# Junacik99/opengl-ray-tracer

Hardware: AMD Instinct MI355X
Metric: Mrays/sec + FPS @1920x1080, car scene (4122 shapes), 1/2/4/8 GPUs (higher is better)
Workload: dtype f32

## Files before the change

### opengl-ray-tracer_amd/csrc/rt_device.h

```cpp
#pragma once

#include <hip/hip_runtime.h>
#include <stdint.h>

namespace rtd {

struct GeoRec {
    int type, idx;
    float f[18];
};
static_assert(sizeof(GeoRec) == 80, "GeoRec is 5 float4");

struct PrimRec {
    float f[15];
    int st;
};
static_assert(sizeof(PrimRec) == 64, "PrimRec is 4 float4");
__device__ __forceinline__ int prim_type(const PrimRec& g) { return g.st & 3; }

struct V {
    float x, y, z;
};
__host__ __device__ __forceinline__ V mk(float x, float y, float z) { return V{x, y, z}; }
__host__ __device__ __forceinline__ V operator+(V a, V b) { return V{a.x + b.x, a.y + b.y, a.z + b.z}; }
// ... 29 lines not shown
    int S, N, I;
    int max_stack;
    V cam_pos, cam_front, cam_right, cam_up;
    float plane_w, plane_h;
    V light_pos, light_color;
    float resX, resY;
    int maxBounces, useBVH, useFresnel, useMT;
    int width, height, y0, stripe, period, out_rows;
    char* __restrict__ dst;
    size_t pitch;
    unsigned long long* __restrict__ stats;
    unsigned long long* __restrict__ tile_times;
    int tiles_x, tiles;
    const int* __restrict__ tile_order;
    int lane_k, lane_k_mode;
    int heavy_k, heavy_parts;
    unsigned* __restrict__ tile_cost;
    int cost_time;
    unsigned long long* __restrict__ heavy_acc;
    unsigned* __restrict__ sched_hist;
    int lane_from_depth;
    int shadow_lane_from;
    int root_ok;
    float root_lo[3], root_hi[3];
    int lane_stack;
    float4* __restrict__ tail_queue;
    int* __restrict__ tail_px;
    int* __restrict__ tail_count;
    int* __restrict__ tail_count_next;
    int tail_from;
    int tail_rx, tail_regions;
    int tail_counters;
    int tail_max_lanes;
    int rgb;
    float shadow_off;
    int ss;
};

__device__ __forceinline__ int image_row(const KParams& kp, int r) {
    return kp.y0 + r + (r / kp.stripe) * (kp.period - kp.stripe);
}

__device__ __forceinline__ Ray get_ray(const KParams& kp, float ndcX, float ndcY) {
    V p = ((kp.cam_pos + kp.cam_front) + (ndcX * kp.plane_w / 2.0f) * kp.cam_right) +
          (ndcY * kp.plane_h / 2.0f) * kp.cam_up;
    return Ray{kp.cam_pos, normalize(p - kp.cam_pos)};
}

struct Hit {
    int type;
    V p;
};

__device__ __forceinline__ Hit intersect(const GeoRec& g, const Ray& r, int use_mt) {
    Hit h{NONE, V{0.f, 0.f, 0.f}};
    const float* f = g.f;
    if (g.type == 0) {
        V c = mk(f[0], f[1], f[2]);
        V oc = r.o - c;
        float aa = dot(r.d, r.d);
        float bb = 2.0f * dot(r.d, oc);
        float cc = dot(oc, oc) - f[3] * f[3];
        float D = bb * bb - 4.0f * aa * cc;
        if (D > 0.0f) {
            float sD = __builtin_sqrtf(D);
            float t1 = (-bb - sD) / (2.0f * aa);
// ... 163 lines not shown
```

### opengl-ray-tracer_amd/csrc/rt_kernels.hip

```cpp
#include <hip/hip_runtime.h>

#include <algorithm>
#include <chrono>
#include <climits>
#include <cmath>
#include <cstdio>
#include <cstdlib>
#include <cstring>
#include <functional>
#include <limits>
#include <atomic>
#include <memory>
#include <new>
#include <thread>
#include <vector>

#include "../../include/rt_api.h"
#include "accel.h"
#include "accel_math.h"
#include "lbvh.h"
#include "rt_device.h"
#include "group_wait.h"
#include "rt_internal.h"

using namespace rtd;

namespace {

constexpr int kBlock = 256;
constexpr int kTileW = 32;
constexpr int kTileH = 8;
constexpr int kMaxStack = 64;
constexpr int kRing = 1024;
constexpr int kLeafScan = 8;

enum {
    ST_PIXELS = 0, ST_CLOSEST, ST_SHADOW, ST_NODES,
    ST_BVH0, ST_BVH1, ST_BVH2, ST_BVH3,
    ST_BR0, ST_BR1, ST_BR2, ST_BR3,
    ST_UPD, ST_HITS, ST_COUNT
};


__device__ GeoRec pack_geo(const FlatShape& s, int si) {
    GeoRec g;
    for (int k = 0; k < 18; ++k) g.f[k] = 0.f;
    g.type = s.type;
    g.idx = si;
    if (s.type == RT_SPHERE) {
        g.f[0] = s.sphereCenter.x; g.f[1] = s.sphereCenter.y; g.f[2] = s.sphereCenter.z;
        g.f[3] = s.sphereRadius;
    } else {
        V n = mk(s.planeNormal.x, s.planeNormal.y, s.planeNormal.z);
        g.f[0] = n.x; g.f[1] = n.y; g.f[2] = n.z; g.f[3] = s.planeD;
        if (s.type == RT_WALL) {
            g.f[4] = s.wallStart.x; g.f[5] = s.wallStart.y; g.f[6] = s.wallStart.z;
// ... 831 lines not shown
        const int ci = k.code[i], cj = k.code[j];
        k.t[i] = sw ? tj : ti, k.t[j] = sw ? ti : tj;
        k.code[i] = sw ? cj : ci, k.code[j] = sw ? ci : cj;
    };
    cx(0, 1), cx(2, 3), cx(4, 5), cx(6, 7), cx(0, 2), cx(1, 3), cx(4, 6), cx(5, 7), cx(1, 2), cx(5, 6);
    cx(0, 4), cx(1, 5), cx(2, 6), cx(3, 7), cx(2, 4), cx(3, 5), cx(1, 2), cx(3, 4), cx(5, 6);
    return k;
}
__device__ __forceinline__ int pick_code8(const Kids8& k, int i) {
    int r = k.code[0];
#pragma unroll
    for (int s2 = 1; s2 < 8; ++s2) r = i == s2 ? k.code[s2] : r;
    return r;
}
__device__ __forceinline__ float pick_t8(const Kids8& k, int i) {
    float r = k.t[0];
#pragma unroll
    for (int s2 = 1; s2 < 8; ++s2) r = i == s2 ? k.t[s2] : r;
    return r;
}

__device__ __forceinline__ int pick_code(const Kids4& k, int i) {
    return i == 0 ? k.code[0] : i == 1 ? k.code[1] : i == 2 ? k.code[2] : k.code[3];
}
__device__ __forceinline__ float pick_t(const Kids4& k, int i) {
    return i == 0 ? k.t[0] : i == 1 ? k.t[1] : i == 2 ? k.t[2] : k.t[3];
}

__device__ __forceinline__ unsigned short f_bf16_down(float t) {
    return static_cast<unsigned short>(__float_as_uint(t) >> 16);
}
__device__ __forceinline__ float bf16_f(unsigned short b) { return __uint_as_float(static_cast<unsigned>(b) << 16); }

template <bool SHADOW, bool COUNT = false, bool WSTAT = false, bool MT = false, bool FLAT_SHADOW = false>
__device__ void lane_walk(const AccelPtrs& A, const Ray& r, bool active, float lim_shadow, Best& b, bool& shadow,
                          int* stk, unsigned short* stt, int stride, int cap, WalkCount& wc, int sg = 1,
                          int si = 0) {
    if (A.N <= 0 || !active) return;
    const V inv = inv_dir(r.d);
    const bool fast = A.boxes_finite && aabb_fast_ok(r.o, inv);
    const rta::RayC c = ray_c<MT>(r, A);
    float tl = rta::t_limit(SHADOW ? lim_shadow : b.d, c.rdl);
    int sp = 0, cur = A.troot;
    const int capo = cap * stride;
    bool have = true;
    bool ovf = false;
    int pcap = min(cap, A.scene_stack) * stride;
    unsigned fm = 0;
    if (!use_scene(A, fast, c)) {
        have = enter_root(A, r, inv, c, tl, cur);
        pcap = capo;
    } else if (A.nfew > 0) {
        fm = few_mask(A, r, inv);
    }
    int start = 0, count = 0;
    if (sg > 1) {
        const float tl0 = SHADOW ? tl : INFINITY;
        int ss = sg;
        while (have && ss > 1) {
            const unsigned uc = static_cast<unsigned>(cur);
            if (uc & (kLeaf | kItem)) break;
            if (COUNT) wc.nodes++;
            if (uc & kTopLeaf) {
                if (count > 0) break;
                const int4 lf = A.tleaf[uc & 0x0fffffffu];
                start = lf.x;
                count = lf.y;
                have = lf.z != kNoChild;
                cur = lf.z;
            } else if (uc & kLocal) {
                if constexpr (!MT && kWide8) {
                    const Kids8 w = sort8(wide_kids<MT>(A, uc, c, tl0, true), wide_kids_hi<MT>(A, uc, c, tl0, true));
                    int h = 0;
#pragma unroll
                    for (int s2 = 0; s2 < 8; ++s2) h += w.t[s2] < INFINITY;
                    if (h == 0) {
                        have = false;
                    } else if (h >= ss) {
                        for (int q = si + ss; q < h; q += ss) {
                            if (sp < pcap) {
                                stk[sp] = pick_code8(w, q);
                                stt[sp] = f_bf16_down(pick_t8(w, q));
                                sp += stride;
                            } else {
                                ovf = true;
                            }
                        }
// ... 17 lines not shown
                                stk[sp] = pick_code(w, si + ss);
                                stt[sp] = f_bf16_down(pick_t(w, si + ss));
                                sp += stride;
                            } else {
                                ovf = true;
                            }
                        }
                        cur = pick_code(w, si);
                        ss = 1;
                    } else {
                        const int p = si * h / ss, lo = (p * ss + h - 1) / h, hi = ((p + 1) * ss + h - 1) / h;
                        cur = pick_code(w, p);
                        si -= lo;
                        ss = hi - lo;
                    }
                }
            } else {
                const Kids k = ref_kids(A, uc, r, inv, c, tl0, true, fast);
                if (k.ha && k.hb) {
                    const bool a_first = !(k.tb < k.ta);
                    const int p = si * 2 / ss, lo = (p * ss + 1) / 2, hi = ((p + 1) * ss + 1) / 2;
                    cur = (p == 0) == a_first ? k.ca : k.cb;
                    si -= lo;
                    ss = hi - lo;
                } else if (k.ha || k.hb) {
                    cur = k.ha ? k.ca : k.cb;
                } else {
                    have = false;
                }
            }
        }
    }
    if (!have) cur = kNoChild;
    bool ended = false;
    for (;;) {
        bool stop = ended;
        for (;;) {
            if (__ballot(!stop && count == 0) == 0) break;
            if (!stop && cur == kNoChild) {
                if (sp == 0) {
                    if (ovf) {
                        ovf = false;
                        pcap = capo;
                        if (!enter_root(A, r, inv, c, tl, cur)) cur = kNoChild;
                    }
                    if (cur == kNoChild) {
                        ended = count == 0;
                        stop = true;
                    }
                } else {
                    sp -= stride;
                    const int pc = stk[sp];
                    cur = bf16_f(stt[sp]) > tl ? kNoChild : pc;
                }
            }
            const unsigned uc = static_cast<unsigned>(cur);
            stop = stop || (cur != kNoChild && count > 0 && (uc & (kTopLeaf | kLeaf)));
            if (stop || cur == kNoChild) continue;
            if (COUNT) wc.nodes++;
            if (WSTAT && first_active()) wc.wnodes++;
            cur = kNoChild;
            if (uc & kLocal) {
                if (uc & kLeaf) {
                    start = static_cast<int>((uc >> 6) & 0x3fffffu);
                    count = static_cast<int>(uc & 0x3fu);
                    if (uc & kItem) count = ((fm >> (count >> 3)) & 1u) ? (count & 7) : 0;
                } else {
                    auto push = [&](float t, int code) {
// ... 26 lines not shown
                        const bool vf = vt < w.t[0];
                        push(vf ? w.t[0] : vt, vf ? w.code[0] : vc);
                        w.t[0] = vf ? vt : w.t[0];
                        w.code[0] = vf ? vc : w.code[0];
                    }
                    if (w.t[0] < INFINITY) cur = w.code[0];
                }
            } else if ((uc & (kTopLeaf | kItem)) == (kTopLeaf | kItem)) {
                int s0, n0;
                if (enter_item(A, uc, r, inv, s0, n0)) {
                    start = s0;
                    count = n0;
                }
            } else if (uc & kTopLeaf) {
                const int4 lf = A.tleaf[uc & 0x0fffffffu];
                start = lf.x;
                count = lf.y;
                cur = lf.z;
            } else {
                const Kids k = ref_kids(A, uc, r, inv, c, tl, true, fast);
                if (k.ha && k.hb) {
                    const bool a_first = !(k.tb < k.ta);
                    if (sp < capo) {
                        stk[sp] = a_first ? k.cb : k.ca;
                        stt[sp] = f_bf16_down(a_first ? k.tb : k.ta);
                        sp += stride;
                    }
                    cur = a_first ? k.ca : k.cb;
                } else if (k.ha || k.hb) {
                    cur = k.ha ? k.ca : k.cb;
                }
            }
        }
        if (__ballot(count > 0) == 0) return;
        for (int i = 0; i < count; ++i) {
            const PrimRec g = load_prim(A.prims, start + i);
            if (COUNT) wc.tests++;
            if (WSTAT && first_active()) wc.wtests++;
            if (SHADOW && FLAT_SHADOW) {
                if (try_shadow<MT>(g, r, lim_shadow)) {
                    shadow = true;
                    ended = true;
                    count = i + 1;
                }
            } else if (SHADOW) {
                if (try_shadow<MT>(g, r, lim_shadow)) {
                    shadow = true;
                    if (sg == 1) return;
                    ended = true;
                    break;
                }
            } else {
                try_closest<MT>(g, start + i, r, b);
            }
        }
        count = 0;
        if (sg > 1) {
            if (SHADOW) {
                int any = shadow ? 1 : 0;
                for (int o = 1; o < sg; o <<= 1) any |= __shfl_xor(any, o);
                if (any) {
                    shadow = true;
                    ended = true;
                }
            } else {
                float d = b.d;
                for (int o = 1; o < sg; o <<= 1) d = fminf(d, __shfl_xor(d, o));
// ... 203 lines not shown
            const float ra = __int_as_float(__builtin_amdgcn_readlane(__float_as_int(k.ta), rep));
            const float rb = __int_as_float(__builtin_amdgcn_readlane(__float_as_int(k.tb), rep));
            const bool a_first = !(rb < ra);
            if (st.sp < kMaxStack) st.push(a_first ? k.cb : k.ca, a_first ? mb : ma);
            cur = a_first ? k.ca : k.cb;
            m = a_first ? ma : mb;
        } else if (ma) {
            cur = k.ca;
            m = ma;
        } else if (mb) {
            cur = k.cb;
            m = mb;
        } else {
            m = 0;
        }
    }
}

__device__ __forceinline__ PixelCoord tile_pixel(const KParams& kp, int tile) {
    const int lane = threadIdx.x & 63;
    PixelCoord pc;
    pc.x = (tile % kp.tiles_x) * 8 + (lane & 7);
    pc.r = (tile / kp.tiles_x) * 8 + (lane >> 3);
    pc.active = pc.x < kp.width && pc.r < kp.out_rows;
    pc.y = pc.active ? image_row(kp, pc.r) : 0;
    pc.active = pc.active && pc.y < kp.height;
    return pc;
}

constexpr int kTileRec = 24;

constexpr int kTailRegion = 64 * 64;
constexpr size_t kTailAutoItems = 8192;

constexpr int kOrderBuckets = 32, kOrderThreads = 256;
constexpr int kSplitMax = 16, kSplitGroup = 8;
constexpr int kMtWalkFrom = 1 << 16;
constexpr int kMtPacketMaxNodes = 1024;
constexpr int kHeavyTiles = -1, kHeavyParts = 4, kHeavyAutoSlots = 2;
constexpr int kLatencyMaxSlots = 12;
constexpr unsigned kXcds = 8;

__device__ __forceinline__ int work_bucket(unsigned c) {
    if (c < 2u) return 0;
    const int l = 31 - __builtin_clz(c);
    return min(kOrderBuckets - 1, 2 * l - 1 + static_cast<int>((c >> (l - 1)) & 1u));
}

__device__ __forceinline__ unsigned long long wave_sum(unsigned long long v) {
    for (int off = 32; off > 0; off >>= 1) v += __shfl_xor(v, off);
    return v;
}

__device__ __forceinline__ void walk_rec(unsigned long long* rec, int slot, const WalkCount& before,
                                         const WalkCount& after, unsigned long long ticks) {
    if (!rec || slot >= 8) return;
    const unsigned long long n = wave_sum(after.nodes - before.nodes);
    if ((threadIdx.x & 63) == 0) {
        rec[6 + slot] = ticks;
        rec[14 + slot] = n;
    }
}

template <bool COUNT, bool COST, bool MT, bool SPLIT, class BgY>
__device__ __forceinline__ void bounce_step(const AccelPtrs& A, const float4* __restrict__ mat, const KParams& kp,
                                            int depth, Ray& ray, bool& alive, V& acc, V& att, BgY bg_y, int* stk,
// ... 168 lines not shown
                o[4] = mn;
                o[5] = mt;
            }
        }
        if (REC && kp.tile_cost) {
            const unsigned long long work = !COST || kp.cost_time
                                                ? (wall_clock64() - t0) >> 2
                                                : wave_sum(static_cast<unsigned long long>(wc.nodes) + wc.tests);
            unsigned wk = static_cast<unsigned>(work < 0xffffffffull ? work : 0xffffffffull);
            bool rec = part == 0;
            if (part > 0 && lane == 0) {
                const int hk = slot / kp.heavy_parts;
                const unsigned long long old =
                    atomicAdd(&kp.heavy_acc[hk], (1ull << 56) | static_cast<unsigned long long>(wk));
                if (static_cast<int>(old >> 56) == kp.heavy_parts - 1) {
                    const unsigned long long sum = (old & ((1ull << 56) - 1)) + wk;
                    wk = static_cast<unsigned>(sum < 0xffffffffull ? sum : 0xffffffffull);
                    rec = true;
                }
            }
            if (lane == 0 && rec) {
                kp.tile_cost[tile] = wk;
                atomicAdd(&kp.sched_hist[(tile / kOrderThreads) * kOrderBuckets + work_bucket(wk)], 1u);
            }
        }
    }
}

__device__ __forceinline__ int wave_sum_int(int v) {
    for (int off = 32; off > 0; off >>= 1) v += __shfl_xor(v, off);
    return v;
}

__global__ __launch_bounds__(kBlock) RT_ACCEL_ATTR void k_accel_tail(AccelPtrs A, const float4* __restrict__ mat,
                                                                      KParams kp) {
    extern __shared__ int lds_stack[];
    int* stk = lds_stack + threadIdx.x;
    unsigned short* stt =
        reinterpret_cast<unsigned short*>(lds_stack + static_cast<size_t>(kp.lane_stack) * blockDim.x) + threadIdx.x;
    const int lane = threadIdx.x & 63;
    int total = 0;
    for (int b = 0; b < kp.tail_regions; b += 64) {
        const int cnt = b + lane < kp.tail_regions ? kp.tail_count[b + lane] : 0;
        total += wave_sum_int((cnt + 63) >> 6);
    }
    const int chunk = blockIdx.x * (blockDim.x >> 6) + (threadIdx.x >> 6);
    if (chunk < total) {
        int rid = 0, first = 0, n = 0, acc0 = 0;
        for (int b = 0; b < kp.tail_regions; b += 64) {
            const int cnt = b + lane < kp.tail_regions ? kp.tail_count[b + lane] : 0;
            const int ch = (cnt + 63) >> 6;
            int incl = ch;
            for (int off = 1; off < 64; off <<= 1) {
                const int y = __shfl_up(incl, off);
                if (lane >= off) incl += y;
            }
            const unsigned long long hit = __ballot(acc0 + incl > chunk && acc0 + incl - ch <= chunk && ch > 0);
            if (hit) {
                const int l = __builtin_ctzll(hit);
                rid = b + l;
                first = __shfl(acc0 + incl - ch, l);
                n = __shfl(cnt, l);
                break;
            }
            acc0 += __shfl(incl, 63);
        }
        const int k = (chunk - first) * 64 + lane;
        bool alive = k < n;
        const int i = rid * kTailRegion + k;
        Ray ray{mk(0.f, 0.f, 0.f), mk(0.f, 0.f, 1.f)};
        V acc = mk(0.f, 0.f, 0.f), att = mk(1.f, 1.f, 1.f);
        int r = 0, x = 0;
        if (alive) {
            const float4* q = kp.tail_queue + 3 * static_cast<size_t>(i);
            const float4 q0 = q[0], q1 = q[1], q2 = q[2];
            const unsigned px = static_cast<unsigned>(kp.tail_px[i]);
            ray = Ray{mk(q0.x, q0.y, q0.z), mk(q1.x, q1.y, q1.z)};
            acc = mk(q0.w, q1.w, q2.w);
            att = mk(q2.x, q2.y, q2.z);
            r = static_cast<int>(px / static_cast<unsigned>(kp.width));
            x = static_cast<int>(px - static_cast<unsigned>(r) * static_cast<unsigned>(kp.width));
        }
        const bool have = alive;
        WalkCount wc{0u, 0u, 0u, 0u};
        for (int depth = kp.tail_from; depth < kp.maxBounces; ++depth) {
            if (__ballot(alive) == 0) break;
            bounce_step<false, false, false, true>(A, mat, kp, depth, ray, alive, acc, att,
                                                   [&]() { return image_row(kp, r); }, stk, stt, kp.lane_stack, wc,
                                                   nullptr, kp.lane_from_depth, kp.shadow_lane_from);
        }
        if (have) store_px(kp, r, x, make_float4(acc.x, acc.y, acc.z, 1.0f));
    }
    if (blockIdx.x == 0)
        for (int b = threadIdx.x; b < kp.tail_counters; b += blockDim.x) kp.tail_count_next[b] = 0;
}

template <int N>
__device__ __forceinline__ float4 box_x(const float4* __restrict__ p) {
    if constexpr (N == 1) {
        return p[0];
    } else {
        const float4 a = box_x<N / 2>(p), b = box_x<N / 2>(p + N / 2);
        return make_float4(a.x + b.x, a.y + b.y, a.z + b.z, a.w + b.w);
    }
}
template <int N, int M>
__device__ __forceinline__ float4 box_y(const char* __restrict__ p, size_t pitch) {
    if constexpr (M == 1) {
        return box_x<N>(reinterpret_cast<const float4*>(p));
    } else {
        const float4 a = box_y<N, M / 2>(p, pitch), b = box_y<N, M / 2>(p + (M / 2) * pitch, pitch);
        return make_float4(a.x + b.x, a.y + b.y, a.z + b.z, a.w + b.w);
    }
}
template <int N>
__global__ __launch_bounds__(256) void k_box_filter(const char* __restrict__ src, size_t src_pitch,
                                                    char* __restrict__ dst, size_t pitch, int width, int height,
                                                    int y0, int stripe, int period, int out_rows, int format) {
    const int x = blockIdx.x * 64 + (threadIdx.x & 63);
    const int r = blockIdx.y * 4 + (threadIdx.x >> 6);
    if (x >= width || r >= out_rows) return;
    const int y = y0 + r + (r / stripe) * (period - stripe);
    if (y >= height) return;
    float4 v = box_y<N, N>(src + static_cast<size_t>(r) * N * src_pitch + static_cast<size_t>(x) * N * sizeof(float4),
// ... 712 lines not shown
    unsigned long long* stats_dev = nullptr;
    int cu_count = 256;
    int lane_from_depth = -1;
    int cone_cull = 1;
    int split_max = kSplitMax, split_g = kSplitGroup;
    int heavy_k = kHeavyTiles, heavy_parts = kHeavyParts;
    int lane_k = -1, lane_k_mode = 2;
    int cost_time = -1;
    int latency_mode = 0;
    int* tile_order = nullptr;
    int tile_order_n = 0;
    int schedule = RT_SCHED_COST;
    unsigned* sched_cost = nullptr;
    unsigned long long* heavy_acc = nullptr;
    size_t heavy_acc_cap = 0;
    int* sched_order = nullptr;
    unsigned* sched_sets = nullptr;
    int sched_parity = 0;
    int sched_cap = 0, sched_valid = 0;
    int sched_period = 16, sched_frame = 0;
    int cost_dilate = 0;
    int moving_period = 1, moving_dilate = 1, moving_split = 0;
    FlatCamera sched_cam{};
    bool have_sched_cam = false;
    bool moving = false;
    unsigned* dil_cost = nullptr;
    size_t dil_cap = 0;
    int tail_from = RT_TAIL_AUTO;
    float4* tail_queue = nullptr;
    size_t tail_cap = 0;
    int* tail_counts = nullptr;
    int tail_regions_cap = 0;
    int tail_max_lanes = 64;
    int shadow_walk_override = -1;
    int tail_parity = 0;
    int lane_stack_override = 0;
    unsigned long long* tile_times = nullptr;
    size_t tile_times_cap = 0;
    std::vector<int> anim_ids;
    std::vector<int> refit_ids;
    std::vector<int> refit_of;
    std::vector<int> anim_cls;
    std::vector<FlatShape> anim_base;
    std::vector<int> upd_ids;
    std::vector<char> upd_mark;
    std::vector<std::pair<int, FlatShape>> upd_base;
    bool nodes_dirty = false;
    bool nodes_rebuild = false;
    bool bounds_rebuild = false;
    int updates_flushed = 0;
    int refit_mode = -1;
    long long direct_reads = 0, n_direct_slot_reads = 0;
    long long dirty_sum = 0;
    long long last_flush_bytes = 0;
    int refit_compactions = 0;
    int dirty_max = 0;
    int* anim_maps = nullptr;
    size_t anim_maps_cap = 0;
    AnimMaps anim{};
    static constexpr int kAnimRing = 3;
    void* anim_pinned[kAnimRing] = {nullptr, nullptr, nullptr};
    void* anim_pinned_dev[kAnimRing] = {nullptr, nullptr, nullptr};
    size_t anim_pinned_cap[kAnimRing] = {0, 0, 0};
    hipEvent_t anim_copied[kAnimRing] = {nullptr, nullptr, nullptr};
    size_t report_at[kAnimRing] = {0, 0, 0};
    bool report_pending[kAnimRing] = {false, false, false};
// ... 1150 lines not shown
        if (rtx::create_ctx(&sub, c->device, c->stream) != RT_OK) return nullptr;
        stale = true;
    }
    return sub;
}

void inherit(rt_ctx* b, const rt_ctx* c) {
    b->cam = c->cam;
    b->light = c->light;
    b->have_cam = b->have_light = true;
    b->params = c->params;
    b->kernel = RT_KERNEL_ACCEL;
    b->lane_from_depth = c->lane_from_depth;
    b->cone_cull = c->cone_cull;
    b->split_max = c->split_max;
    b->split_g = c->split_g;
    b->heavy_k = c->heavy_k;
    b->heavy_parts = c->heavy_parts;
    b->lane_k = c->lane_k;
    b->lane_k_mode = c->lane_k_mode;
    b->cost_time = c->cost_time;
    b->latency_mode = c->latency_mode;
    b->schedule = c->schedule;
    b->sched_period = c->sched_period;
    b->cost_dilate = c->cost_dilate;
    b->moving_period = c->moving_period;
    b->moving_dilate = c->moving_dilate;
    b->moving_split = c->moving_split;
    b->frame_event = c->frame_event;
    b->refit_mode = c->refit_mode;
    b->async_rebuild = c->async_rebuild;
    b->tail_from = c->tail_from;
    b->tail_max_lanes = c->tail_max_lanes;
    b->shadow_walk_override = c->shadow_walk_override;
    b->tree_mode = c->tree_mode;
    b->scene_stack = c->scene_stack;
    b->lane_stack_override = c->lane_stack_override;
    b->ss_general = c->ss_general;
}

int walk_from(const rt_ctx* c) {
    if (c->lane_from_depth >= 0) return c->lane_from_depth;
    return c->accel.mt && c->N < kMtPacketMaxNodes ? kMtWalkFrom : 1;
}

bool sub_usable(const rt_ctx* b, const KParams& kp) {
    const float cmag = std::max({std::fabs(kp.cam_pos.x), std::fabs(kp.cam_pos.y), std::fabs(kp.cam_pos.z)});
    return b->accel_ok && cmag <= b->accel.origin_lim;
}

rt_ctx* brute_ctx(rt_ctx* c, const KParams& kp) {
    if (!c->brute_accel || kp.useBVH || c->S <= 0 ||
        (c->kernel != RT_KERNEL_AUTO && c->kernel != RT_KERNEL_ACCEL))
        return nullptr;
    rt_ctx* b = sub_ctx(c, c->brute, c->brute_stale);
    if (!b) return nullptr;
    if (c->brute_stale) {
        FlatNode leaf;
        std::memset(&leaf, 0, sizeof leaf);
        const float inf = std::numeric_limits<float>::infinity();
        leaf.boundsMin = rt_vec3{-inf, -inf, -inf};
        leaf.boundsMax = rt_vec3{inf, inf, inf};
        leaf.leftChild = leaf.rightChild = -1;
        leaf.startShapeIdx = 0;
        leaf.numShapes = c->S;
        std::vector<int> order(c->S);
// ... 243 lines not shown
                }
            }
            const bool stamps_fit =
                !c->tile_times ||
                c->tile_times_cap >= static_cast<size_t>(k2.tiles) + static_cast<size_t>(std::min(hk, k2.tiles)) * hp;
            const bool whole = k2.tile_cost && c->cost_time != 0 && !c->tile_times && latency &&
                               !(c->moving && c->moving_split);
            const bool blocks_whole = !ss_fused || hp * k2.ss <= 8;
            if (stamps_fit && hp > 1 && hk > 0 && !whole && blocks_whole) {
                k2.heavy_k = std::min(hk, k2.tiles);
                k2.heavy_parts = hp;
            }
        }
        k2.cost_time = c->cost_time != 0 ? 1 : 0;
        k2.heavy_acc = nullptr;
        if (k2.tile_cost && k2.heavy_k > 0) {
            const size_t need = static_cast<size_t>(k2.heavy_k);
            if (c->heavy_acc_cap < need) {
                hipFree(c->heavy_acc);
                c->heavy_acc = nullptr;
                c->heavy_acc_cap = 0;
                if (hipMalloc(&c->heavy_acc, need * sizeof(unsigned long long)) != hipSuccess) return RT_ERR_NO_MEMORY;
                c->heavy_acc_cap = need;
            }
            HIP_TRY(hipMemsetAsync(c->heavy_acc, 0, need * sizeof(unsigned long long), c->stream));
            k2.heavy_acc = c->heavy_acc;
        }
        const int troot = c->tree_mode == RT_TREE_SCENE && !c->st_suspended ? c->st_root : kNoChild;
        const AccelPtrs A{c->anodes, c->prims, c->lnodes, c->wnodes, c->tleaf, c->titems, troot,
                          c->scene_stack > 0 ? c->scene_stack : kMaxStack, c->nfew, kp.N, c->accel.origin_lim,
                          c->boxes_finite, c->split_max, c->split_g, c->prim_idx_dev,
                          {c->accel.mt_z[0], c->accel.mt_z[1], c->accel.mt_z[2]}};
        k2.tail_queue = nullptr;
        const int tail_from = c->tail_from != RT_TAIL_AUTO
                                  ? c->tail_from
                                  : (c->accel.st.item_ref.size() >= kTailAutoItems ? 2 : 0);
        const bool tail = tail_from > 0 && tail_from < k2.maxBounces && !ss_fused &&
                          static_cast<unsigned long long>(k2.width) * k2.out_rows < (1ull << 32);
        const int rx = (k2.tiles_x + 7) / 8, regions = rx * ((k2.tiles / k2.tiles_x + 7) / 8);
        if (tail) {
            const size_t need = static_cast<size_t>(regions) * kTailRegion;
            if (need > c->tail_cap) {
                hipFree(c->tail_queue);
                c->tail_queue = nullptr;
                c->tail_cap = 0;
                if (hipMalloc(&c->tail_queue, need * (3 * sizeof(float4) + sizeof(int))) != hipSuccess)
                    return RT_ERR_NO_MEMORY;
                c->tail_cap = need;
            }
            if (regions > c->tail_regions_cap) {
                hipFree(c->tail_counts);
                c->tail_counts = nullptr;
                c->tail_regions_cap = 0;
                if (hipMalloc(&c->tail_counts, 2 * static_cast<size_t>(regions) * sizeof(int)) != hipSuccess)
                    return RT_ERR_NO_MEMORY;
                HIP_TRY(hipMemsetAsync(c->tail_counts, 0, 2 * static_cast<size_t>(regions) * sizeof(int), c->stream));
                c->tail_regions_cap = regions;
            }
            k2.tail_queue = c->tail_queue;
            k2.tail_px = reinterpret_cast<int*>(c->tail_queue + 3 * c->tail_cap);
            k2.tail_count = c->tail_counts + c->tail_parity * c->tail_regions_cap;
            k2.tail_count_next = c->tail_counts + (1 - c->tail_parity) * c->tail_regions_cap;
            k2.tail_from = tail_from;
            k2.tail_rx = rx;
            k2.tail_regions = regions;
            k2.tail_counters = c->tail_regions_cap;
            k2.tail_max_lanes = c->tail_max_lanes;
        }
        auto kfn = k_accel<false>;
        if (c->accel.mt) {
            k2.tail_queue = nullptr;
            kfn = !k2.tile_cost  ? k_accel<false, false, false, true>
                  : k2.cost_time ? k_accel<false, false, false, true, true>
                                 : k_accel<false, true, false, true>;
        } else if (c->tile_times) {
            k2.tail_queue = nullptr;
            kfn = k_accel<true>;
        } else if (tail) {
            kfn = !k2.tile_cost  ? k_accel<false, false, true>
                  : k2.cost_time ? k_accel<false, false, true, false, true>
                                 : k_accel<false, true, true>;
        } else if (latency) {
            kfn = !k2.tile_cost  ? k_accel<false, false, true, false, false, false>
                  : k2.cost_time ? k_accel<false, false, true, false, true, false>
                                 : k_accel<false, true, true, false, true, false>;
        } else if (!k2.tile_cost) {
            kfn = k_accel<false, false>;
        } else if (k2.cost_time) {
            kfn = k_accel<false, false, false, false, true>;
        }
        if (ss_fused) {
            if (c->accel.mt)
                kfn = !k2.tile_cost  ? k_accel<false, false, false, true, false, false, true>
                      : k2.cost_time ? k_accel<false, false, false, true, true, false, true>
                                     : k_accel<false, true, false, true, true, false, true>;
            else if (latency)
                kfn = !k2.tile_cost  ? k_accel<false, false, true, false, false, false, true>
                      : k2.cost_time ? k_accel<false, false, true, false, true, false, true>
                                     : k_accel<false, true, true, false, true, false, true>;
            else
                kfn = !k2.tile_cost  ? k_accel<false, false, false, false, false, false, true>
                      : k2.cost_time ? k_accel<false, false, false, false, true, false, true>
                                     : k_accel<false, true, false, false, true, false, true>;
        }
        const bool tail_on = k2.tail_queue != nullptr;
        const int blocks = k2.tiles + k2.heavy_k * (k2.heavy_parts - 1);
        hipLaunchKernelGGL(kfn, dim3(blocks), dim3(64), lds, c->stream, A, c->mat, k2);
        if (tail_on) {
            const size_t tlds = static_cast<size_t>(k2.lane_stack) * 64 * 6;
            const int tgrid = regions * (kTailRegion / 64);
            hipLaunchKernelGGL(k_accel_tail, dim3(tgrid), dim3(64), tlds, c->stream, A, c->mat, k2);
            c->tail_parity = 1 - c->tail_parity;
        }
        if (ss && !ss_fused) launch_box_filter(c, kin);
        if (k2.tile_cost) {
            if (rec) HIP_TRY(hipEventRecord(e1, c->stream));
            order_after = true;
            const unsigned* set = c->sched_sets + c->sched_parity * sched_set_words(c->sched_cap);
            unsigned* next = c->sched_sets + (1 - c->sched_parity) * sched_set_words(c->sched_cap);
            const int groups = (k2.tiles + kOrderThreads - 1) / kOrderThreads;
            const unsigned* cost = c->sched_cost;
            if (latency && c->frame_event) {
                if (!c->frame_ev && hipEventCreateWithFlags(&c->frame_ev, hipEventDisableTiming) != hipSuccess)
                    return RT_ERR_DEVICE;
                HIP_TRY(hipEventRecord(c->frame_ev, c->stream));
                c->frame_ev_set = true;
            }
            if (dilate > 0) {
                const size_t need = static_cast<size_t>(k2.tiles) + static_cast<size_t>(groups) * kOrderBuckets;
                if (c->dil_cap < need) {
                    hipFree(c->dil_cost);
                    c->dil_cost = nullptr;
                    c->dil_cap = 0;
                    if (hipMalloc(&c->dil_cost, need * sizeof(unsigned)) != hipSuccess) return RT_ERR_NO_MEMORY;
                    c->dil_cap = need;
                }
                hipLaunchKernelGGL(k_cost_dilate, dim3(groups), dim3(kOrderThreads), 0, c->stream, c->sched_cost,
                                   k2.tiles, k2.tiles_x, dilate, c->dil_cost, c->dil_cost + k2.tiles);
                cost = c->dil_cost;
                set = c->dil_cost + k2.tiles;
            }
            hipLaunchKernelGGL(k_tile_order, dim3(groups), dim3(kOrderThreads),
                               0, c->stream, cost, k2.tiles, set, next,
                               static_cast<int>(sched_set_words(c->sched_cap)), c->sched_order,
// ... 136 lines not shown
    if (c->brute && !c->brute_stale)
        for (int i = 0; i < n && !c->brute_stale; ++i)
            if (rt_update_shapes(c->brute, c->anim_ids[i], 1, &shapes[i]) != RT_OK) c->brute_stale = true;
    if (c->mtc && !c->mtc_stale && rtx::animate_deferred(c->mtc, shapes) != RT_OK) c->mtc_stale = true;
    return RT_OK;
}

bool rtx::view_root(const rt_ctx* c, float lo[3], float hi[3]) {
    if (!c || !c->have_scene || c->N <= 0) return false;
    std::memcpy(lo, c->root_lo, sizeof c->root_lo);
    std::memcpy(hi, c->root_hi, sizeof c->root_hi);
    return true;
}

extern "C" {

int rt_destroy(rt_ctx* c) {
    if (!c) return RT_ERR_INVALID;
    hipSetDevice(c->device);
    if (c->stream) sync_stream(c);
    if (c->brute) rt_destroy(c->brute);
    c->brute = nullptr;
    if (c->mtc) rt_destroy(c->mtc);
    c->mtc = nullptr;
    free_scene(c);
    hipFree(c->staging_shapes);
    hipFree(c->staging_nodes);
    hipFree(c->staging_idx);
    hipFree(c->img);
    hipFree(c->ss_buf);
    hipFree(c->stats_dev);
    hipFree(c->tail_queue);
    hipFree(c->tail_counts);
    hipFree(c->tile_times);
    hipFree(c->tile_order);
    hipFree(c->sched_cost);
    hipFree(c->dil_cost);
    hipFree(c->heavy_acc);
    hipFree(c->sched_order);
    hipFree(c->sched_sets);
    hipFree(c->anim_maps);
    hipFree(c->anim_sbox);
    for (int k = 0; k < rt_ctx::kAnimRing; ++k) {
        if (c->anim_pinned[k]) hipHostFree(c->anim_pinned[k]);
        if (c->anim_copied[k]) hipEventDestroy(c->anim_copied[k]);
    }
    for (hipEvent_t e : c->ring0) if (e) hipEventDestroy(e);
    for (hipEvent_t e : c->ring1) if (e) hipEventDestroy(e);
    if (c->sync_ev) hipEventDestroy(c->sync_ev);
    if (c->frame_ev) hipEventDestroy(c->frame_ev);
    if (c->ev0) hipEventDestroy(c->ev0);
    if (c->ev1) hipEventDestroy(c->ev1);
    if (c->own_stream && c->stream) hipStreamDestroy(c->stream);
    delete c;
    return RT_OK;
}

int rt_set_stream(rt_ctx* c, void* s) {
    if (!c) return RT_ERR_INVALID;
    if (set_dev(c) != RT_OK) return RT_ERR_DEVICE;
    if (const int rc = record_mark(c)) return rc;
    HIP_TRY(sync_stream(c));
    if (c->own_stream) hipStreamDestroy(c->stream);
    if (s) {
        c->stream = static_cast<hipStream_t>(s);
        c->own_stream = false;
// ... 609 lines not shown
    return RT_OK;
}

extern "C" int rt_set_walk(rt_ctx* c, int lane_from_depth) {
    if (!c || lane_from_depth < -1) return RT_ERR_INVALID;
    c->lane_from_depth = lane_from_depth;
    return RT_OK;
}

extern "C" int rt_debug_cone_cull(rt_ctx* c, int on) {
    if (!c) return RT_ERR_INVALID;
    c->cone_cull = on ? 1 : 0;
    return c->have_scene ? upload_accel(c) : RT_OK;
}

extern "C" int rt_debug_scene_stack(rt_ctx* c, int n) {
    if (!c || n < 0) return RT_ERR_INVALID;
    c->scene_stack = n;
    return RT_OK;
}

extern "C" int rt_debug_shadow_walk(rt_ctx* c, int from) {
    if (!c || from < -1) return RT_ERR_INVALID;
    c->shadow_walk_override = from;
    return RT_OK;
}

extern "C" int rt_debug_tail_lanes(rt_ctx* c, int lanes) {
    if (!c || lanes < 0 || lanes > 64) return RT_ERR_INVALID;
    c->tail_max_lanes = lanes;
    return RT_OK;
}

extern "C" int rt_set_tail(rt_ctx* c, int from_bounce) {
    if (!c || from_bounce < RT_TAIL_AUTO) return RT_ERR_INVALID;
    c->tail_from = from_bounce;
    return RT_OK;
}

extern "C" int rt_debug_sched_period(rt_ctx* c, int period) {
    if (!c || period < 1) return RT_ERR_INVALID;
    c->sched_period = period;
    c->sched_frame = 0;
    return RT_OK;
}

extern "C" int rt_debug_moving(rt_ctx* c, int period, int dilate, int split) {
    if (!c || period < 0 || dilate < 0 || dilate > 64) return RT_ERR_INVALID;
    c->moving_period = period;
    c->moving_dilate = dilate;
    c->moving_split = split ? 1 : 0;
    return RT_OK;
}

extern "C" int rt_debug_frame_event(rt_ctx* c, int on) {
    if (!c || on < 0 || on > 1) return RT_ERR_INVALID;
    c->frame_event = on;
    return RT_OK;
}

extern "C" int rt_debug_cost_dilate(rt_ctx* c, int r) {
    if (!c || r < 0 || r > 64) return RT_ERR_INVALID;
    c->cost_dilate = r;
    return RT_OK;
}

// ... 117 lines not shown
```

### opengl-ray-tracer_amd/rtamd.py

```python
from __future__ import annotations

import ctypes as C
import os
from dataclasses import dataclass

import numpy as np

HERE = os.path.dirname(os.path.abspath(__file__))
LIBDIR = os.environ.get("RTAMD_LIBDIR") or os.path.join(HERE, "lib")


def _vec(off):
    return [("x", off), ("y", off + 4), ("z", off + 8)]


MATERIAL_DTYPE = np.dtype({
    "names": ["color", "fresnelStrength", "ambientStrength", "diffuseStrength", "specularStrength", "shininess"],
    "formats": [("<f4", 3), "<f4", "<f4", "<f4", "<f4", "<i4"],
    "offsets": [0, 12, 16, 20, 24, 28],
    "itemsize": 32,
})

SHAPE_DTYPE = np.dtype({
    "names": ["type", "material", "sphereCenter", "sphereRadius", "planeNormal", "planeD",
# ... 590 lines not shown
    def read_tree(self):
        _, n, i = self.scene_size()
        nodes = np.zeros(n, NODE_DTYPE)
        idx = np.zeros(i, np.int32)
        if n:
            self._chk(self._lib.rt_read_nodes(self._h, _ptr(nodes), n), "rt_read_nodes")
        self._chk(self._lib.rt_read_indices(self._h, _ptr(idx) if i else None, i), "rt_read_indices")
        return nodes, idx

    def set_tree(self, mode):
        self._chk(self._lib.rt_set_tree(self._h, int(mode)), "rt_set_tree")

    def set_tail(self, from_bounce):
        self._chk(self._lib.rt_set_tail(self._h, int(from_bounce)), "rt_set_tail")

    def set_samples(self, n):
        self._chk(self._lib.rt_set_samples(self._h, int(n)), "rt_set_samples")

    def debug_ss_general(self, on):
        fn = self._lib.rt_debug_ss_general
        fn.argtypes = [_P, _I]
        self._chk(fn(self._h, int(bool(on))), "rt_debug_ss_general")

    def debug_shadow_walk(self, from_bounce):
        fn = self._lib.rt_debug_shadow_walk
        fn.argtypes = [_P, _I]
        self._chk(fn(self._h, int(from_bounce)), "rt_debug_shadow_walk")

    def debug_tail_lanes(self, lanes):
        fn = self._lib.rt_debug_tail_lanes
        fn.argtypes = [_P, _I]
        self._chk(fn(self._h, int(lanes)), "rt_debug_tail_lanes")

    def set_kernel_timing(self, on):
        self._chk(self._lib.rt_set_kernel_timing(self._h, int(bool(on))), "rt_set_kernel_timing")

    def set_latency_mode(self, on):
        self._chk(self._lib.rt_set_latency_mode(self._h, int(bool(on))), "rt_set_latency_mode")

    def set_schedule(self, mode):
        self._chk(self._lib.rt_set_schedule(self._h, int(mode)), "rt_set_schedule")

    def debug_scene_stack(self, n):
        fn = self._lib.rt_debug_scene_stack
        fn.argtypes = [C.c_void_p, C.c_int]
        self._chk(fn(self._h, int(n)), "rt_debug_scene_stack")

    def debug_sched_period(self, period):
        fn = self._lib.rt_debug_sched_period
        fn.argtypes = [_P, _I]
        self._chk(fn(self._h, int(period)), "rt_debug_sched_period")

    def debug_lane_stack(self, n):
        fn = self._lib.rt_debug_lane_stack
        fn.argtypes = [_P, _I]
        self._chk(fn(self._h, int(n)), "rt_debug_lane_stack")

    def debug_tile_order(self, order):
        fn = self._lib.rt_debug_tile_order
        fn.argtypes = [_P, _P, _I]
        o = np.ascontiguousarray(order if order is not None else [], np.int32)
        self._chk(fn(self._h, _ptr(o) if o.size else None, int(o.size)), "rt_debug_tile_order")

    def debug_anim_rebuilds(self):
        fn = self._lib.rt_debug_anim_rebuilds
        fn.argtypes = [_P]
# ... 296 lines not shown
```

Before: 22760.

## Add persistent-lane ray pool to tail kernel with wavefront refill and compaction

Adds a pooled tail kernel in which each wave owns a chunk of queued rays. Lanes that finish a traversal are refilled with new ray jobs inside lane_walk once enough lanes sit idle, and closest-hit and shadow passes run as separate compacted phases per bounce. The aim is to cut SIMD divergence and idle lanes in incoherent secondary bounces. It is auto-enabled for large scenes with the tail starting at bounce 1, and it adds extra per-ray queue storage (best hit, shadow flag), more global memory traffic and a more complex control path. It also adds a debug stats counter and API.

New measurement: 22770, median of 2. No clear change (+0.1%).

```diff
diff --git a/opengl-ray-tracer_amd/csrc/rt_device.h b/opengl-ray-tracer_amd/csrc/rt_device.h
--- a/opengl-ray-tracer_amd/csrc/rt_device.h
+++ b/opengl-ray-tracer_amd/csrc/rt_device.h
@@ -85,6 +85,10 @@
     int tail_rx, tail_regions;
     int tail_counters;
     int tail_max_lanes;
+    int4* tail_best;
+    int* tail_flag;
+    int tail_pool, tail_idle;
+    unsigned long long* tail_stats;
     int rgb;
     float shadow_off;
     int ss;
diff --git a/opengl-ray-tracer_amd/csrc/rt_kernels.hip b/opengl-ray-tracer_amd/csrc/rt_kernels.hip
--- a/opengl-ray-tracer_amd/csrc/rt_kernels.hip
+++ b/opengl-ray-tracer_amd/csrc/rt_kernels.hip
@@ -22,6 +22,7 @@
 #include "rt_device.h"
 #include "group_wait.h"
 #include "rt_internal.h"
+#include "tail_pool.h"
 
 using namespace rtd;
 
@@ -919,14 +920,53 @@
 }
 __device__ __forceinline__ float bf16_f(unsigned short b) { return __uint_as_float(static_cast<unsigned>(b) << 16); }
 
-template <bool SHADOW, bool COUNT = false, bool WSTAT = false, bool MT = false, bool FLAT_SHADOW = false>
-__device__ void lane_walk(const AccelPtrs& A, const Ray& r, bool active, float lim_shadow, Best& b, bool& shadow,
+struct NoPool {
+    static constexpr bool on = false;
+};
+
+template <bool SHADOW>
+struct TailPool {
+    static constexpr bool on = true;
+    const KParams& kp;
+    const float4* prims;
+    const float4* q;
+    int4* best;
+    int* flag;
+    int next, end, min_idle;
+    unsigned refills;
+    __device__ __forceinline__ void fetch(int job, Ray& r, float& lim, Best& b, bool& shadow) const {
+        const float4 q0 = q[3 * job], q1 = q[3 * job + 1];
+        r = Ray{mk(q0.x, q0.y, q0.z), mk(q1.x, q1.y, q1.z)};
+        shadow = false;
+        if (SHADOW) {
+            const int4 e = best[job];
+            const V hp = hit_point(r, __int_as_float(e.z));
+            const V hn = shape_normal(load_prim(prims, e.w), hp);
+            r = Ray{hp + hn * kp.shadow_off, normalize(kp.light_pos - hp)};
+            lim = gmin(dist(kp.light_pos, hp), 1e20f);
+        } else {
+            b = Best{1e20f, 0x7fffffff, 0.f, -1};
+        }
+    }
+    __device__ __forceinline__ void retire(int job, const Best& b, bool shadow) const {
+        if (SHADOW)
+            flag[job] = shadow ? 1 : 0;
+        else
+            best[job] = make_int4(__float_as_int(b.d), b.seq, __float_as_int(b.t), b.slot);
+    }
+};
+
+template <bool SHADOW, bool COUNT = false, bool WSTAT = false, bool MT = false, bool FLAT_SHADOW = false,
+          class Pool = NoPool>
+__device__ void lane_walk(const AccelPtrs& A, const Ray& r_in, bool active, float lim_shadow, Best& b, bool& shadow,
                           int* stk, unsigned short* stt, int stride, int cap, WalkCount& wc, int sg = 1,
-                          int si = 0) {
-    if (A.N <= 0 || !active) return;
-    const V inv = inv_dir(r.d);
-    const bool fast = A.boxes_finite && aabb_fast_ok(r.o, inv);
-    const rta::RayC c = ray_c<MT>(r, A);
+                          int si = 0, Pool* pool = nullptr) {
+    static_assert(!Pool::on || !SHADOW || FLAT_SHADOW, "a pool's lanes leave the walk together");
+    if (!Pool::on && (A.N <= 0 || !active)) return;
+    std::conditional_t<Pool::on, Ray, const Ray&> r = r_in;
+    std::conditional_t<Pool::on, V, const V> inv = inv_dir(r.d);
+    std::conditional_t<Pool::on, bool, const bool> fast = A.boxes_finite && aabb_fast_ok(r.o, inv);
+    std::conditional_t<Pool::on, rta::RayC, const rta::RayC> c = ray_c<MT>(r, A);
     float tl = rta::t_limit(SHADOW ? lim_shadow : b.d, c.rdl);
     int sp = 0, cur = A.troot;
     const int capo = cap * stride;
@@ -934,12 +974,15 @@
     bool ovf = false;
     int pcap = min(cap, A.scene_stack) * stride;
     unsigned fm = 0;
-    if (!use_scene(A, fast, c)) {
+    if (Pool::on) {
+        have = false;
+    } else if (!use_scene(A, fast, c)) {
         have = enter_root(A, r, inv, c, tl, cur);
         pcap = capo;
     } else if (A.nfew > 0) {
         fm = few_mask(A, r, inv);
     }
+    int job = -1;
     int start = 0, count = 0;
     if (sg > 1) {
         const float tl0 = SHADOW ? tl : INFINITY;
@@ -1023,8 +1066,41 @@
         }
     }
     if (!have) cur = kNoChild;
-    bool ended = false;
+    bool ended = Pool::on;
     for (;;) {
+        if constexpr (Pool::on) {
+            const unsigned long long idle = __ballot(ended);
+            const bool drained = pool->next >= pool->end;
+            if (rtp::refill_now(idle, ~0ull, pool->next, pool->end, pool->min_idle) || (drained && idle == ~0ull)) {
+                if (ended && job >= 0) pool->retire(job, b, shadow);
+                if (drained) return;
+                const int take = rtp::refill_job(idle, lane_id(), pool->next);
+                pool->next = rtp::refill_next(idle, pool->next);
+                pool->refills++;
+                if (ended) {
+                    job = take < pool->end ? take : -1;
+                    if (job >= 0) {
+                        pool->fetch(job, r, lim_shadow, b, shadow);
+                        inv = inv_dir(r.d);
+                        fast = A.boxes_finite && aabb_fast_ok(r.o, inv);
+                        c = ray_c<MT>(r, A);
+                        tl = rta::t_limit(SHADOW ? lim_shadow : b.d, c.rdl);
+                        sp = 0;
+                        cur = A.troot;
+                        ovf = false;
+                        pcap = min(cap, A.scene_stack) * stride;
+                        fm = 0;
+                        if (!use_scene(A, fast, c)) {
+                            if (!enter_root(A, r, inv, c, tl, cur)) cur = kNoChild;
+                            pcap = capo;
+                        } else if (A.nfew > 0) {
+                            fm = few_mask(A, r, inv);
+                        }
+                        ended = false;
+                    }
+                }
+            }
+        }
         bool stop = ended;
         for (;;) {
             if (__ballot(!stop && count == 0) == 0) break;
@@ -1117,7 +1193,10 @@
                 }
             }
         }
-        if (__ballot(count > 0) == 0) return;
+        if (__ballot(count > 0) == 0) {
+            if constexpr (Pool::on) continue;
+            return;
+        }
         for (int i = 0; i < count; ++i) {
             const PrimRec g = load_prim(A.prims, start + i);
             if (COUNT) wc.tests++;
@@ -1387,6 +1466,7 @@
 
 constexpr int kTailRegion = 64 * 64;
 constexpr size_t kTailAutoItems = 8192;
+constexpr int kTailPoolAuto = 256, kRefillIdle = 16, kTailPoolMinSlots = 7;
 
 constexpr int kOrderBuckets = 32, kOrderThreads = 256;
 constexpr int kSplitMax = 16, kSplitGroup = 8;
@@ -1621,6 +1701,47 @@
     return v;
 }
 
+__device__ __forceinline__ bool tail_unit(const KParams& kp, int shift, int unit, int& rid, int& first, int& n) {
+    const int lane = threadIdx.x & 63, per = (1 << shift) - 1;
+    int total = 0;
+    for (int b = 0; b < kp.tail_regions; b += 64) {
+        const int cnt = b + lane < kp.tail_regions ? kp.tail_count[b + lane] : 0;
+        total += wave_sum_int((cnt + per) >> shift);
+    }
+    if (unit >= total) return false;
+    int acc0 = 0;
+    for (int b = 0; b < kp.tail_regions; b += 64) {
+        const int cnt = b + lane < kp.tail_regions ? kp.tail_count[b + lane] : 0;
+        const int ch = (cnt + per) >> shift;
+        int incl = ch;
+        for (int off = 1; off < 64; off <<= 1) {
+            const int y = __shfl_up(incl, off);
+            if (lane >= off) incl += y;
+        }
+        const unsigned long long hit = __ballot(acc0 + incl > unit && acc0 + incl - ch <= unit && ch > 0);
+        if (hit) {
+            const int l = __builtin_ctzll(hit);
+            rid = b + l;
+            first = __shfl(acc0 + incl - ch, l);
+            n = __shfl(cnt, l);
+            return true;
+        }
+        acc0 += __shfl(incl, 63);
+    }
+    return false;
+}
+
+__device__ __forceinline__ void tail_stats_add(const KParams& kp, const WalkCount& wc, unsigned refills,
+                                               unsigned walks) {
+    const unsigned long long v[4] = {wave_sum(wc.nodes), wave_sum(wc.wnodes), wave_sum(wc.tests), wave_sum(wc.wtests)};
+    if ((threadIdx.x & 63) == 0 && kp.tail_stats) {
+        for (int i = 0; i < 4; ++i) atomicAdd(kp.tail_stats + i, v[i]);
+        atomicAdd(kp.tail_stats + 4, static_cast<unsigned long long>(refills));
+        atomicAdd(kp.tail_stats + 5, static_cast<unsigned long long>(walks));
+    }
+}
+
+template <bool STAT>
 __global__ __launch_bounds__(kBlock) RT_ACCEL_ATTR void k_accel_tail(AccelPtrs A, const float4* __restrict__ mat,
                                                                       KParams kp) {
     extern __shared__ int lds_stack[];
@@ -1674,11 +1795,138 @@
         WalkCount wc{0u, 0u, 0u, 0u};
         for (int depth = kp.tail_from; depth < kp.maxBounces; ++depth) {
             if (__ballot(alive) == 0) break;
-            bounce_step<false, false, false, true>(A, mat, kp, depth, ray, alive, acc, att,
+            bounce_step<STAT, false, false, true>(A, mat, kp, depth, ray, alive, acc, att,
                                                    [&]() { return image_row(kp, r); }, stk, stt, kp.lane_stack, wc,
                                                    nullptr, kp.lane_from_depth, kp.shadow_lane_from);
         }
         if (have) store_px(kp, r, x, make_float4(acc.x, acc.y, acc.z, 1.0f));
+        if (STAT) tail_stats_add(kp, wc, 0u, 0u);
+    }
+    if (blockIdx.x == 0)
+        for (int b = threadIdx.x; b < kp.tail_counters; b += blockDim.x) kp.tail_count_next[b] = 0;
+}
+
+template <bool STAT>
+__global__ __launch_bounds__(kBlock) RT_ACCEL_ATTR void k_accel_tail_pool(AccelPtrs A, const float4* __restrict__ mat,
+                                                                           KParams kp) {
+    extern __shared__ int lds_stack[];
+    int* stk = lds_stack + threadIdx.x;
+    unsigned short* stt =
+        reinterpret_cast<unsigned short*>(lds_stack + static_cast<size_t>(kp.lane_stack) * blockDim.x) + threadIdx.x;
+    const int lane = threadIdx.x & 63;
+    const int unit = blockIdx.x * (blockDim.x >> 6) + (threadIdx.x >> 6);
+    const int shift = 31 - __builtin_clz(kp.tail_pool);
+    int rid = 0, first = 0, n = 0;
+    if (tail_unit(kp, shift, unit, rid, first, n)) {
+        const int at = (unit - first) << shift;
+        int cnt = min(kp.tail_pool, n - at);
+        const size_t base = static_cast<size_t>(rid) * kTailRegion + at;
+        float4* q = kp.tail_queue + 3 * base;
+        int* px = kp.tail_px + base;
+        int4* bs = kp.tail_best + base;
+        int* fl = kp.tail_flag + base;
+        const Ray none{mk(0.f, 0.f, 0.f), mk(0.f, 0.f, 1.f)};
+        WalkCount wc{0u, 0u, 0u, 0u};
+        unsigned refills = 0, walks = 0;
+        for (int depth = kp.tail_from; depth < kp.maxBounces && cnt > 0; ++depth) {
+            Best b{1e20f, 0x7fffffff, 0.f, -1};
+            bool sh = false;
+            {
+                TailPool<false> pool{kp, A.prims, q, bs, fl, 0, cnt, kp.tail_idle, 0u};
+                lane_walk<false, STAT, STAT, false, true>(A, none, false, 0.f, b, sh, stk, stt, blockDim.x,
+                                                          kp.lane_stack, wc, 1, 0, &pool);
+                refills += pool.refills;
+                walks += cnt;
+            }
+            __threadfence_block();
+            int w = 0;
+            for (int e0 = 0; e0 < cnt; e0 += 64) {
+                const int e = e0 + lane;
+                const bool valid = e < cnt;
+                float4 q0 = make_float4(0.f, 0.f, 0.f, 0.f), q1 = q0, q2 = q0;
+                int4 be = make_int4(0, 0, 0, -1);
+                int p = 0;
+                if (valid) {
+                    q0 = q[3 * e];
+                    q1 = q[3 * e + 1];
+                    q2 = q[3 * e + 2];
+                    p = px[e];
+                    be = bs[e];
+                }
+                const bool hit = valid && be.w >= 0;
+                if (valid && !hit) {
+                    const int r = static_cast<int>(static_cast<unsigned>(p) / static_cast<unsigned>(kp.width));
+                    const int x = static_cast<int>(static_cast<unsigned>(p) -
+                                                   static_cast<unsigned>(r) * static_cast<unsigned>(kp.width));
+                    const V acc =
+                        mk(q0.w, q1.w, q2.w) + mulv(mk(q2.x, q2.y, q2.z), background(kp, image_row(kp, r)));
+                    store_px(kp, r, x, make_float4(acc.x, acc.y, acc.z, 1.0f));
+                }
+                const unsigned long long keep = __ballot(hit);
+                const int d = rtp::compact_slot(keep, lane, w);
+                if (hit && d != e) {
+                    q[3 * d] = q0;
+                    q[3 * d + 1] = q1;
+                    q[3 * d + 2] = q2;
+                    px[d] = p;
+                    bs[d] = be;
+                }
+                w += rtp::popc(keep);
+            }
+            cnt = w;
+            if (cnt == 0) break;
+            __threadfence_block();
+            {
+                TailPool<true> pool{kp, A.prims, q, bs, fl, 0, cnt, kp.tail_idle, 0u};
+                lane_walk<true, STAT, STAT, false, true>(A, none, false, 0.f, b, sh, stk, stt, blockDim.x,
+                                                         kp.lane_stack, wc, 1, 0, &pool);
+                refills += pool.refills;
+                walks += cnt;
+            }
+            __threadfence_block();
+            const bool last = depth + 1 >= kp.maxBounces;
+            w = 0;
+            for (int e0 = 0; e0 < cnt; e0 += 64) {
+                const int e = e0 + lane;
+                const bool valid = e < cnt;
+                Ray ray = none;
+                V acc = mk(0.f, 0.f, 0.f), att = mk(1.f, 1.f, 1.f);
+                int p = 0;
+                bool alive = false;
+                if (valid) {
+                    const float4 q0 = q[3 * e], q1 = q[3 * e + 1], q2 = q[3 * e + 2];
+                    const int4 be = bs[e];
+                    const bool shadow = fl[e] != 0;
+                    p = px[e];
+                    ray = Ray{mk(q0.x, q0.y, q0.z), mk(q1.x, q1.y, q1.z)};
+                    acc = mk(q0.w, q1.w, q2.w);
+                    att = mk(q2.x, q2.y, q2.z);
+                    const PrimRec g = load_prim(A.prims, be.w);
+                    const V hp = hit_point(ray, __int_as_float(be.z));
+                    alive = shade_bounce(kp, ray, hp, shape_normal(g, hp), load_mat(mat, A.prim_shape[be.w]), shadow,
+                                         acc, att, 1e-3f);
+                }
+                const bool on = alive && !last;
+                if (valid && !on) {
+                    const int r = static_cast<int>(static_cast<unsigned>(p) / static_cast<unsigned>(kp.width));
+                    const int x = static_cast<int>(static_cast<unsigned>(p) -
+                                                   static_cast<unsigned>(r) * static_cast<unsigned>(kp.width));
+                    store_px(kp, r, x, make_float4(acc.x, acc.y, acc.z, 1.0f));
+                }
+                const unsigned long long keep = __ballot(on);
+                if (on) {
+                    const int d = rtp::compact_slot(keep, lane, w);
+                    q[3 * d] = make_float4(ray.o.x, ray.o.y, ray.o.z, acc.x);
+                    q[3 * d + 1] = make_float4(ray.d.x, ray.d.y, ray.d.z, acc.y);
+                    q[3 * d + 2] = make_float4(att.x, att.y, att.z, acc.z);
+                    px[d] = p;
+                }
+                w += rtp::popc(keep);
+            }
+            cnt = w;
+            __threadfence_block();
+        }
+        if (STAT) tail_stats_add(kp, wc, refills, walks);
     }
     if (blockIdx.x == 0)
         for (int b = threadIdx.x; b < kp.tail_counters; b += blockDim.x) kp.tail_count_next[b] = 0;
@@ -2457,6 +2705,9 @@
     int* tail_counts = nullptr;
     int tail_regions_cap = 0;
     int tail_max_lanes = 64;
+    bool tail_has_pool = false;
+    int tail_pool = -1, tail_idle = kRefillIdle;
+    unsigned long long* tail_stats = nullptr;
     int shadow_walk_override = -1;
     int tail_parity = 0;
     int lane_stack_override = 0;
@@ -3673,6 +3924,8 @@
     b->async_rebuild = c->async_rebuild;
     b->tail_from = c->tail_from;
     b->tail_max_lanes = c->tail_max_lanes;
+    b->tail_pool = c->tail_pool;
+    b->tail_idle = c->tail_idle;
     b->shadow_walk_override = c->shadow_walk_override;
     b->tree_mode = c->tree_mode;
     b->scene_stack = c->scene_stack;
@@ -3982,21 +4235,27 @@
                           c->boxes_finite, c->split_max, c->split_g, c->prim_idx_dev,
                           {c->accel.mt_z[0], c->accel.mt_z[1], c->accel.mt_z[2]}};
         k2.tail_queue = nullptr;
-        const int tail_from = c->tail_from != RT_TAIL_AUTO
-                                  ? c->tail_from
-                                  : (c->accel.st.item_ref.size() >= kTailAutoItems ? 2 : 0);
+        const bool pool_auto = c->tail_from == RT_TAIL_AUTO && c->tail_pool < 0 && !c->latency_mode &&
+                               c->accel.st.item_ref.size() >= kTailAutoItems &&
+                               k2.tiles >= kTailPoolMinSlots * std::max(1, c->cu_count) * 16;
+        const int tail_from = pool_auto                       ? 1
+                              : c->tail_from != RT_TAIL_AUTO ? c->tail_from
+                              : (c->accel.st.item_ref.size() >= kTailAutoItems ? 2 : 0);
+        const int tail_pool = pool_auto ? kTailPoolAuto : std::max(0, c->tail_pool);
+        const int tail_idle = pool_auto ? kRefillIdle : c->tail_idle;
         const bool tail = tail_from > 0 && tail_from < k2.maxBounces && !ss_fused &&
                           static_cast<unsigned long long>(k2.width) * k2.out_rows < (1ull << 32);
         const int rx = (k2.tiles_x + 7) / 8, regions = rx * ((k2.tiles / k2.tiles_x + 7) / 8);
         if (tail) {
             const size_t need = static_cast<size_t>(regions) * kTailRegion;
-            if (need > c->tail_cap) {
+            if (need > c->tail_cap || (tail_pool > 0 && !c->tail_has_pool)) {
                 hipFree(c->tail_queue);
                 c->tail_queue = nullptr;
                 c->tail_cap = 0;
-                if (hipMalloc(&c->tail_queue, need * (3 * sizeof(float4) + sizeof(int))) != hipSuccess)
-                    return RT_ERR_NO_MEMORY;
+                const size_t per = 3 * sizeof(float4) + sizeof(int) + (tail_pool > 0 ? sizeof(int4) + sizeof(int) : 0);
+                if (hipMalloc(&c->tail_queue, need * per) != hipSuccess) return RT_ERR_NO_MEMORY;
                 c->tail_cap = need;
+                c->tail_has_pool = tail_pool > 0;
             }
             if (regions > c->tail_regions_cap) {
                 hipFree(c->tail_counts);
@@ -4008,7 +4267,12 @@
                 c->tail_regions_cap = regions;
             }
             k2.tail_queue = c->tail_queue;
-            k2.tail_px = reinterpret_cast<int*>(c->tail_queue + 3 * c->tail_cap);
+            k2.tail_best = reinterpret_cast<int4*>(c->tail_queue + 3 * c->tail_cap);
+            k2.tail_px = reinterpret_cast<int*>(k2.tail_best + (c->tail_has_pool ? c->tail_cap : 0));
+            k2.tail_flag = k2.tail_px + c->tail_cap;
+            k2.tail_pool = tail_pool;
+            k2.tail_idle = tail_idle;
+            k2.tail_stats = c->tail_stats;
             k2.tail_count = c->tail_counts + c->tail_parity * c->tail_regions_cap;
             k2.tail_count_next = c->tail_counts + (1 - c->tail_parity) * c->tail_regions_cap;
             k2.tail_from = tail_from;
@@ -4058,8 +4322,10 @@
         hipLaunchKernelGGL(kfn, dim3(blocks), dim3(64), lds, c->stream, A, c->mat, k2);
         if (tail_on) {
             const size_t tlds = static_cast<size_t>(k2.lane_stack) * 64 * 6;
-            const int tgrid = regions * (kTailRegion / 64);
-            hipLaunchKernelGGL(k_accel_tail, dim3(tgrid), dim3(64), tlds, c->stream, A, c->mat, k2);
+            const int tgrid = regions * (kTailRegion / (tail_pool > 0 ? tail_pool : 64));
+            auto tfn = tail_pool > 0 ? (k2.tail_stats ? k_accel_tail_pool<true> : k_accel_tail_pool<false>)
+                                     : (k2.tail_stats ? k_accel_tail<true> : k_accel_tail<false>);
+            hipLaunchKernelGGL(tfn, dim3(tgrid), dim3(64), tlds, c->stream, A, c->mat, k2);
             c->tail_parity = 1 - c->tail_parity;
         }
         if (ss && !ss_fused) launch_box_filter(c, kin);
@@ -4262,6 +4528,7 @@
     hipFree(c->stats_dev);
     hipFree(c->tail_queue);
     hipFree(c->tail_counts);
+    hipFree(c->tail_stats);
     hipFree(c->tile_times);
     hipFree(c->tile_order);
     hipFree(c->sched_cost);
@@ -4937,6 +5204,35 @@
     return RT_OK;
 }
 
+extern "C" int rt_debug_tail_pool(rt_ctx* c, int pool, int idle) {
+    if (!c || pool < -1 || idle < 1 || idle > 64) return RT_ERR_INVALID;
+    if (pool > 0 && (pool < 64 || pool > kTailRegion || (pool & (pool - 1)))) return RT_ERR_INVALID;
+    c->tail_pool = pool;
+    c->tail_idle = idle;
+    return RT_OK;
+}
+
+extern "C" int rt_debug_tail_stats(rt_ctx* c, int on, unsigned long long* out) {
+    if (!c) return RT_ERR_INVALID;
+    HIP_TRY(hipSetDevice(c->device));
+    if (out) {
+        for (int i = 0; i < 6; ++i) out[i] = 0;
+        if (c->tail_stats) {
+            HIP_TRY(hipStreamSynchronize(c->stream));
+            HIP_TRY(hipMemcpy(out, c->tail_stats, 6 * sizeof(unsigned long long), hipMemcpyDeviceToHost));
+        }
+    }
+    if (on && !c->tail_stats && hipMalloc(&c->tail_stats, 6 * sizeof(unsigned long long)) != hipSuccess)
+        return RT_ERR_NO_MEMORY;
+    if (!on && c->tail_stats) {
+        HIP_TRY(hipStreamSynchronize(c->stream));
+        hipFree(c->tail_stats);
+        c->tail_stats = nullptr;
+    }
+    if (c->tail_stats) HIP_TRY(hipMemsetAsync(c->tail_stats, 0, 6 * sizeof(unsigned long long), c->stream));
+    return RT_OK;
+}
+
 extern "C" int rt_set_tail(rt_ctx* c, int from_bounce) {
     if (!c || from_bounce < RT_TAIL_AUTO) return RT_ERR_INVALID;
     c->tail_from = from_bounce;
diff --git a/opengl-ray-tracer_amd/csrc/tail_pool.h b/opengl-ray-tracer_amd/csrc/tail_pool.h
--- /dev/null
+++ b/opengl-ray-tracer_amd/csrc/tail_pool.h
@@ -0,0 +1,28 @@
+#ifndef RT_TAIL_POOL_H
+#define RT_TAIL_POOL_H
+
+#if defined(__HIPCC__) || defined(__CUDACC__)
+#define RT_POOL_HD __host__ __device__ inline
+#else
+#define RT_POOL_HD inline
+#endif
+
+namespace rtp {
+
+RT_POOL_HD int popc(unsigned long long m) { return __builtin_popcountll(m); }
+
+RT_POOL_HD int rank_below(unsigned long long m, int lane) { return popc(m & ((1ull << lane) - 1ull)); }
+
+RT_POOL_HD bool refill_now(unsigned long long idle, unsigned long long lanes, int next, int end, int min_idle) {
+    return next < end && (popc(idle) >= min_idle || idle == lanes);
+}
+
+RT_POOL_HD int refill_job(unsigned long long idle, int lane, int next) { return next + rank_below(idle, lane); }
+
+RT_POOL_HD int refill_next(unsigned long long idle, int next) { return next + popc(idle); }
+
+RT_POOL_HD int compact_slot(unsigned long long keep, int lane, int w) { return w + rank_below(keep, lane); }
+
+}
+
+#endif
diff --git a/opengl-ray-tracer_amd/rtamd.py b/opengl-ray-tracer_amd/rtamd.py
--- a/opengl-ray-tracer_amd/rtamd.py
+++ b/opengl-ray-tracer_amd/rtamd.py
@@ -646,6 +646,19 @@
         fn.argtypes = [_P, _I]
         self._chk(fn(self._h, int(lanes)), "rt_debug_tail_lanes")
 
+    def debug_tail_pool(self, pool, idle=32):
+        fn = self._lib.rt_debug_tail_pool
+        fn.argtypes = [_P, _I, _I]
+        self._chk(fn(self._h, int(pool), int(idle)), "rt_debug_tail_pool")
+
+    def debug_tail_stats(self, on=True):
+        fn = self._lib.rt_debug_tail_stats
+        fn.argtypes = [_P, _I, _P]
+        out = (C.c_ulonglong * 6)()
+        self._chk(fn(self._h, int(bool(on)), C.cast(out, _P)), "rt_debug_tail_stats")
+        return dict(zip(("lane_nodes", "wave_nodes", "lane_tests", "wave_tests", "refills", "walks"),
+                        (int(v) for v in out)))
+
     def set_kernel_timing(self, on):
         self._chk(self._lib.rt_set_kernel_timing(self._h, int(bool(on))), "rt_set_kernel_timing")
 
```
